# kvas7andy/unreal

Measured on AMD Instinct MI355X. Metric: env-steps/sec (whole node), UNREAL maze 84x84, higher is better.
Workload: dtype f32 (fp16x2-split MFMA operands, fp32 accumulate)

## Files before the change

### include/unreal_hip.h

```cpp
#ifndef UNREAL_HIP_H
#define UNREAL_HIP_H
#include <stdint.h>
#ifdef __cplusplus
extern "C" {
#endif

#define UNREAL_FRAME_BYTES 21168
#define UNREAL_PC_CELLS 400
#define UNREAL_GEMM_RELU 1
#define UNREAL_GEMM_ACCUM 2
#define UNREAL_GEMM_ATOMIC 4
#define UNREAL_GEMM_RELU_MASK 8
#define UNREAL_GEMM_RELU_BITS 16

int unreal_maze_step(int B, int H1, const int* actions, const int* active, int* pos, int* last_action,
                     float* last_reward, int* count, uint8_t* frames, float* r_reward, int* r_action,
                     int* r_terminal, int* r_last_action, float* r_last_reward, float* r_pc,
                     float* out_reward, int* out_terminal, float* episode_reward, float* score_out,
                     int* score_valid, int reset_on_terminal, int track_score, void* stream);
int unreal_maze_rollout_step(int B, int H1, const int* actions, int* pos, int* last_action, float* last_reward, int* count,
                             uint8_t* frames, float* r_reward, int* r_action, int* r_terminal, int* r_last_action,
                             float* r_last_reward, float* r_pc, float* out_reward, int* out_terminal,
                             float* episode_reward, float* score_out, int* score_valid, int* active,
                             int* active_log_t, int* n_steps, int* terminal_end, int* next_idx ,
// ... 162 lines not shown
                       const float* bv, const double* u, float* pi_out, float* v_out, int* action, void* stream);
int unreal_base_loss_grad(int rows, int A, const float* pi, int ld_pi, const float* v, const int* action,
                          const float* adv, const float* R, const int* active, float entropy_beta, float grad_scale,
                          float* dlogits, float* dv, float* losses , void* stream);
int unreal_vr_loss_grad(int rows, const float* v, const float* R, const int* mask, float grad_scale, float* dv,
                        float* loss, void* stream);
int unreal_rp_loss_grad(int rows, const float* logits, const int* cls, float grad_scale, float* prob, float* dlogits,
                        float* loss, void* stream);
int unreal_colsum(int rows, int cols, const float* X, int ld, float* out, void* stream);
int unreal_relu_mask(int rows, int cols, float* d, int ldd, const float* src, int lds, void* stream);

int unreal_pc_deconv_fwd(int N, int A, const float* hp, const float* hp_absmax, const float* Wv, const float* bv,
                         const float* Wa, const float* ba, float* qmax, const int* action, const float* target,
                         const int* mask, float lambda, float grad_scale, float* d_dec, float* ddec_absmax, float* loss,
                         void* stream);
int unreal_pc_deconv_bwd(int N, int A, const float* hp, const float* hp_absmax, const float* d_dec, const float* ddec_absmax,
                         const float* Wv, const float* Wa, float* d_hp, float* dhp_absmax ,
                         float* dWv, float* dbv, float* dWa, float* dba, void* stream);
int unreal_pc_deconv_train(int N, int A, const float* hp, const float* hp_absmax, const float* Wv, const float* bv,
                           const float* Wa, const float* ba, const int* action, const float* target, const int* mask,
                           float lambda, float grad_scale, float* loss, float* d_hp,
                           float* dhp_absmax , float* dWv, float* dbv, float* dWa,
                           float* dba, float* d_dec, void* stream);

int unreal_grad_norm(const float* grad, long n, float* scratch , float* norm_out, void* stream);
int unreal_rmsprop_step(float* var, float* ms, float* mom, const float* grad, long n, float lr, float decay,
                        float momentum, float eps, float clip_norm, const float* norm, void* stream);

int unreal_copy_words(long n, const void* src, void* dst, void* stream);
int unreal_axpy_f32(long n, float alpha, const float* x, float* y, void* stream);
int unreal_last_launch(char* buf, int len, void* stream);

#ifdef __cplusplus
}
#endif
#endif
```

### unreal_amd/csrc/pc.hip

```cpp
#include "common.h"

namespace {

constexpr int HP_LD = 36, HP_ROWS = 84;
constexpr int NPLP = 2;
constexpr int WD_ELEMS = 4 * 4 * 2 * 4 * 16 * 4;
constexpr int HP_V = (C2_POS * 8 + 255) / 256;
constexpr int DD_V = (PC_CELLS * 8 / 4 + 255) / 256;

struct PcFwdArgs {
  int N, A;
  const float* hp;
  const float* hp_absmax;
  const float* Wv; const float* bv; const float* Wa; const float* ba;
  float* qmax;
  const int* action;
  const float* target;
  const int* mask;
  float lambda, grad_scale;
  float* d_dec;
  float* ddec_absmax;
  float* loss;
};

// ... 5 lines not shown
}

__device__ __forceinline__ void hp_load(const float* __restrict__ src, int gtid, f32x4 (&r)[HP_V]) {
  const f32x4* s4 = reinterpret_cast<const f32x4*>(src);
#pragma unroll
  for (int c = 0; c < HP_V; ++c) {
    int id = gtid + 256 * c;
    r[c] = s4[id < C2_POS * 8 ? id : gtid];
  }
}

__device__ __forceinline__ void hp_store(float* hp, int gtid, const f32x4 (&r)[HP_V]) {
#pragma unroll
  for (int c = 0; c < HP_V; ++c) {
    int id = gtid + 256 * c;
    if (id < C2_POS * 8) *reinterpret_cast<f32x4*>(hp + (id >> 3) * HP_LD + (id & 7) * 4) = r[c];
  }
}

typedef _Float16 fh8p __attribute__((ext_vector_type(8)));
typedef _Float16 fh2p __attribute__((ext_vector_type(2)));
typedef float f32x2p __attribute__((ext_vector_type(2)));
typedef unsigned int u32x2p __attribute__((ext_vector_type(2)));

constexpr int HPP_ROW = 80;
constexpr int HPP_PLANE = HP_ROWS * HPP_ROW;
constexpr int WDP_ROW = 80;
constexpr int WDP_PLANE = 4 * 32 * WDP_ROW;

__device__ __forceinline__ void split4p(const f32x4& v, float scale, u32x2p (&pl)[NPLP]) {
  const f32x2p x01 = (f32x2p){v[0], v[1]} * scale, x23 = (f32x2p){v[2], v[3]} * scale;
  const fh2p h01 = __builtin_convertvector(x01, fh2p), h23 = __builtin_convertvector(x23, fh2p);
  const fh2p l01 = __builtin_convertvector(x01 - __builtin_convertvector(h01, f32x2p), fh2p);
  const fh2p l23 = __builtin_convertvector(x23 - __builtin_convertvector(h23, f32x2p), fh2p);
  pl[0] = (u32x2p){__builtin_bit_cast(unsigned int, h01), __builtin_bit_cast(unsigned int, h23)};
  pl[1] = (u32x2p){__builtin_bit_cast(unsigned int, l01), __builtin_bit_cast(unsigned int, l23)};
}

__device__ __forceinline__ void hp_store_planes(unsigned char* hpp, int gtid, const f32x4 (&r)[HP_V], float scale) {
#pragma unroll
  for (int c = 0; c < HP_V; ++c) {
    const int id = gtid + 256 * c;
    if (id < C2_POS * 8) {
      u32x2p pl[NPLP];
      split4p(r[c], scale, pl);
      pl[0][0] = keep_positive_visible(pl[0][0], r[c][0], r[c][1]);
// ... 37 lines not shown
      for (int k = 0; k < 4; ++k) v[k] = deconv_w(Wv, Wa, A, ky, kx, co, 4 * c4 + k);
    }
    u32x2p pl[NPLP];
    split4p(v, S_W, pl);
#pragma unroll
    for (int t = 0; t < NPLP; ++t) *reinterpret_cast<u32x2p*>(wdp + t * WDP_PLANE + (dd * 32 + n) * WDP_ROW + c4 * 8) = pl[t];
  }
}

__device__ __forceinline__ void pc_zero_hp_pad_rows(unsigned char* hpp) {
  for (int e = threadIdx.x; e < NPLP * 3 * HPP_ROW / 4; e += 256) {
    const int t = e / (3 * HPP_ROW / 4), w = e % (3 * HPP_ROW / 4);
    reinterpret_cast<uint32_t*>(hpp + t * HPP_PLANE + C2_POS * HPP_ROW)[w] = 0u;
  }
}

template <int COT> struct FwdLds {
  static constexpr int DS = COT | 1;
  static constexpr int DEC = NPLP * HPP_PLANE, DOUT = DEC + PC_CELLS * DS * 4, W = DOUT + PC_CELLS * COT * 4,
                       BYTES = W + NPLP * WDP_PLANE;
  static constexpr int WGS = 3 * BYTES <= 160 * 1024 ? 3 : 2;
};

template <bool TWO_NT, int DS>
__device__ __forceinline__ void deconv_packed(const unsigned char* hpp, const unsigned char* wdp, float* dec, int mt0, int i,
                                              int q, int CO, const float (&bias)[2], float unscale) {
  constexpr int NTL = TWO_NT ? 2 : 1;
  const int ntiles = (mt0 + 4 < 7) ? 2 : 1;
  f32x4 acc[2][NTL];
  int a[2], b[2];
#pragma unroll
  for (int t = 0; t < 2; ++t) {
#pragma unroll
    for (int nt = 0; nt < NTL; ++nt) acc[t][nt] = (f32x4){0.f, 0.f, 0.f, 0.f};
    const int m = min((mt0 + 4 * t) * 16 + i, 99);
    a[t] = m / 10;
    b[t] = m % 10;
  }
#pragma unroll
  for (int dd = 0; dd < 4; ++dd) {
    const int da = dd >> 1, db = dd & 1;
    fh8p bw[NTL][NPLP];
#pragma unroll
    for (int nt = 0; nt < NTL; ++nt)
#pragma unroll
      for (int pl = 0; pl < NPLP; ++pl)
        bw[nt][pl] = *reinterpret_cast<const fh8p*>(wdp + pl * WDP_PLANE + ((dd * 32 + nt * 16 + i)) * WDP_ROW + 16 * q);
#pragma unroll
    for (int t = 0; t < 2; ++t) {
      if (t < ntiles) {
        const int y = a[t] - da, x = b[t] - db;
        const int row = (y >= 0 && y < 9 && x >= 0 && x < 9) ? y * 9 + x : C2_POS;
        fh8p av[NPLP];
#pragma unroll
        for (int pl = 0; pl < NPLP; ++pl)
          av[pl] = *reinterpret_cast<const fh8p*>(hpp + pl * HPP_PLANE + row * HPP_ROW + 16 * q);
#pragma unroll
        for (int nt = 0; nt < NTL; ++nt) PC_SPLIT_MMA(av, bw[nt], acc[t][nt]);
      }
    }
  }
#pragma unroll
  for (int nt = 0; nt < NTL; ++nt) {
    const int n = nt * 16 + i;
    if (n < 4 * CO) {
      const int par = n / CO, co = n - par * CO;
#pragma unroll
      for (int t = 0; t < 2; ++t)
        if (t < ntiles) {
#pragma unroll
// ... 49 lines not shown
  }
  int prev = -1;
  for (int base = blockIdx.x; base < p.N; base += stride) {
    const int n = base;
    const bool valid = n < p.N;
    const int nn = n + stride;
    const bool has_next = nn < p.N;
    __syncthreads();
    if (prev >= 0 && p.d_dec) {
      f32x4* dst = reinterpret_cast<f32x4*>(p.d_dec + (size_t)prev * PC_CELLS * CO);
      for (int id = gtid; id < PC_CELLS * CO / 4; id += 256) dst[id] = reinterpret_cast<const f32x4*>(dout)[id];
    }
    if (has_next) hp_load(p.hp + (size_t)nn * F2_DIM, gtid, pre);
    float tg[2] = {0.f, 0.f};
    int act = 0;
    bool on = true;
    if (valid && p.d_dec) {
      tg[0] = p.target[(size_t)n * PC_CELLS + gtid];
      tg[1] = p.target[(size_t)n * PC_CELLS + min(gtid + 256, PC_CELLS - 1)];
      act = p.action[n];
      on = p.mask[n] != 0;
    }
    if (valid) {
      if (two_nt) deconv_packed<true, DS>(hpp, wdp, dec, gw, i, q, CO, bias, unscale);
      else deconv_packed<false, DS>(hpp, wdp, dec, gw, i, q, CO, bias, unscale);
    }
    __syncthreads();
    if (valid) {
#pragma unroll
      for (int pi = 0; pi < 2; ++pi) {
        const int pos = gtid + 256 * pi;
        if (pos >= PC_CELLS) break;
        const float* d = dec + pos * DS;
        const float vpre = d[0];
        const float V = fmaxf(vpre, 0.f);
        float adv[8], mean = 0.f;
        for (int k = 0; k < A; ++k) { adv[k] = fmaxf(d[1 + k], 0.f); mean += adv[k]; }
        mean /= (float)A;
        if (p.qmax) {
          float mx = V + adv[0] - mean;
          for (int k = 1; k < A; ++k) mx = fmaxf(mx, V + adv[k] - mean);
          p.qmax[(size_t)n * PC_CELLS + pos] = mx;
        }
        if (p.d_dec) {
          const float qa = V + adv[act] - mean;
          const float diff = tg[pi] - qa;
          const float dq = on ? -p.lambda * diff * p.grad_scale : 0.f;
          if (on) loss_acc += 0.5f * p.lambda * diff * diff;
// ... 67 lines not shown
    const int k = e & 31, ci = (e >> 5) & 31, ky = e >> 10;
    const int kx = k >> 3, co = k & 7;
    float v = 0.f;
    if (co == 0) v = Wv[(ky * 4 + kx) * 32 + ci];
    else if (co <= A) v = Wa[((ky * 4 + kx) * A + (co - 1)) * 32 + ci];
    unsigned short t[NPLP];
    split1p(v, S_W, t);
#pragma unroll
    for (int pl = 0; pl < NPLP; ++pl)
      reinterpret_cast<unsigned short*>(wbp + pl * WBP_PLANE + (ky * 32 + ci) * WDP_ROW)[k] = t[pl];
  }
}

__device__ __forceinline__ void pc_stage_dd(unsigned char* ddp, int gtid, const float (&dd)[2][8], float S_DD, float (&adbk)[8]) {
#pragma unroll
  for (int h = 0; h < 2; ++h) {
    const int pos = gtid + 256 * h;
    if (pos < PC_CELLS) {
      u32x2p lo[NPLP], hi[NPLP];
      split4p((f32x4){dd[h][0], dd[h][1], dd[h][2], dd[h][3]}, S_DD, lo);
      split4p((f32x4){dd[h][4], dd[h][5], dd[h][6], dd[h][7]}, S_DD, hi);
#pragma unroll
      for (int pl = 0; pl < NPLP; ++pl) {
        typedef unsigned int u32x4p __attribute__((ext_vector_type(4)));
        *reinterpret_cast<u32x4p*>(ddp + pl * DDP_PLANE + pos * DDP_ROW) = (u32x4p){lo[pl][0], lo[pl][1], hi[pl][0], hi[pl][1]};
      }
#pragma unroll
      for (int k = 0; k < 8; ++k) adbk[k] += dd[h][k];
    }
  }
}

__device__ __forceinline__ void pc_dgrad_frame(const unsigned char* hpp, const unsigned char* ddp, const unsigned char* wbp,
                                               float* dhs, int gw, int i, int q, float un_dgrad) {
  const int nt = gw & 1;
  f32x4 acc[3];
  int abase[3];
#pragma unroll
  for (int jj = 0; jj < 3; ++jj) {
    acc[jj] = (f32x4){0.f, 0.f, 0.f, 0.f};
    const int pos = min(((gw >> 1) + 2 * jj) * 16 + i, C2_POS - 1);
    abase[jj] = ((2 * (pos / 9)) * 20 + 2 * (pos % 9) + q) * DDP_ROW;
  }
#pragma unroll
  for (int ky = 0; ky < 4; ++ky) {
    fh8p bw[NPLP];
#pragma unroll
    for (int pl = 0; pl < NPLP; ++pl)
      bw[pl] = *reinterpret_cast<const fh8p*>(wbp + pl * WBP_PLANE + (ky * 32 + nt * 16 + i) * WDP_ROW + 16 * q);
#pragma unroll
    for (int jj = 0; jj < 3; ++jj) {
      fh8p av[NPLP];
#pragma unroll
      for (int pl = 0; pl < NPLP; ++pl)
        av[pl] = *reinterpret_cast<const fh8p*>(ddp + pl * DDP_PLANE + abase[jj] + ky * 20 * DDP_ROW);
      PC_SPLIT_MMA(av, bw, acc[jj]);
    }
  }
#pragma unroll
  for (int jj = 0; jj < 3; ++jj)
#pragma unroll
    for (int r = 0; r < 4; ++r) {
      const int pos = ((gw >> 1) + 2 * jj) * 16 + 4 * q + r;
      if (pos < C2_POS) {
        const int ci = nt * 16 + i;
        const unsigned short h0 = reinterpret_cast<const unsigned short*>(hpp + pos * HPP_ROW)[ci];
        dhs[pos * 32 + ci] = (h0 != 0 && !(h0 & 0x8000)) ? acc[jj][r] * un_dgrad : 0.f;
      }
    }
}

__device__ __forceinline__ void pc_wgrad_frame(const unsigned char* hpp, const unsigned char* ddp, int gw, int i, int q,
// ... 111 lines not shown
#pragma unroll
      for (int co = 0; co < 8; ++co) pre_dd[h][co] = (co < CO) ? src[pos * CO + co] : 0.f;
    }
  };

  __syncthreads();
  {
    const int n0 = blockIdx.x;
    if (n0 < p.N) {
      hp_load(p.hp + (size_t)n0 * F2_DIM, gtid, pre_hp);
      hp_store_planes(hpp, gtid, pre_hp, S_HP);
      load_dd(n0);
      pc_stage_dd(ddp, gtid, pre_dd, S_DD, adbk);
    }
  }
  for (int n = blockIdx.x; n < p.N; n += stride) {
    const int nn = n + stride;
    const bool has_next = nn < p.N;
    __syncthreads();
    if (has_next) {
      hp_load(p.hp + (size_t)nn * F2_DIM, gtid, pre_hp);
      load_dd(nn);
    }
    pc_dgrad_frame(hpp, ddp, wbp, dhs, gw, i, q, un_dgrad);
    pc_wgrad_frame(hpp, ddp, gw, i, q, aw);
    __syncthreads();
    dhp_max = pc_drain_dhp(dhs, p.d_hp + (size_t)n * F2_DIM, gtid, dhp_max);
    if (has_next) {
      hp_store_planes(hpp, gtid, pre_hp, S_HP);
      pc_stage_dd(ddp, gtid, pre_dd, S_DD, adbk);
    }
  }
  pc_commit_grads(aw, un_wgrad, adbk, dhp_max, A, p.dWv, p.dWa, p.dbv, p.dba, p.dhp_absmax, s_red, gw, lane, i, q);
}

struct PcTrainArgs {
  int N, A;
  const float* hp; const float* hp_absmax;
  const float* Wv; const float* bv; const float* Wa; const float* ba;
  const int* action; const float* target; const int* mask;
  float lambda, grad_scale;
  float* loss;
  float* d_hp; float* dhp_absmax;
  float* dWv; float* dbv; float* dWa; float* dba;
  float* d_dec;
};

template <int COT> struct TrainLds {
  static constexpr int DS = COT | 1;
  static constexpr int UNI = PC_CELLS * DS * 4 > F2_DIM * 4 ? PC_CELLS * DS * 4 : F2_DIM * 4;
  static constexpr int DDP = NPLP * HPP_PLANE, U = DDP + NPLP * DDP_PLANE, WF = U + UNI, WB = WF + NPLP * WDP_PLANE,
                       RED = WB + NPLP * WBP_PLANE, BYTES = RED + 192;
  static constexpr int WGS = 2 * BYTES <= 160 * 1024 ? 2 : 1;
};

template <int COT>
__global__ __launch_bounds__(256, TrainLds<COT>::WGS) void pc_deconv_train_kernel(PcTrainArgs p) {
  typedef TrainLds<COT> L;
  constexpr int DS = L::DS;
  __shared__ __attribute__((aligned(16))) unsigned char smem[L::BYTES];
  const int gtid = threadIdx.x;
  const int lane = threadIdx.x & 63, gw = gtid >> 6;
  const int i = lane & 15, q = lane >> 4;
  unsigned char* hpp = smem;
  unsigned char* ddp = smem + L::DDP;
  float* uni = reinterpret_cast<float*>(smem + L::U);
  unsigned char* wdp = smem + L::WF;
  unsigned char* wbp = smem + L::WB;
  float* red = reinterpret_cast<float*>(smem + L::RED);
  const int A = p.A, CO = 1 + p.A;

  const float S_W = pow2_scale(pc_weight_max(p.Wv, p.Wa, A, red));
  const float S_HP = pow2_scale(*p.hp_absmax);
  const float un_fwd = pow2_inv(S_HP) * pow2_inv(S_W);
  pc_fwd_weight_planes(p.Wv, p.Wa, A, wdp, S_W);
  pc_bwd_weight_planes(p.Wv, p.Wa, A, wbp, S_W);
  pc_zero_hp_pad_rows(hpp);
  for (int e = gtid; e < NPLP * DDP_PLANE / 4; e += 256) reinterpret_cast<uint32_t*>(ddp)[e] = 0u;
  float bias[2];
#pragma unroll
  for (int nt = 0; nt < 2; ++nt) {
    const int n = nt * 16 + i;
    const int co = n % CO;
    bias[nt] = (n < 4 * CO) ? (co == 0 ? p.bv[0] : p.ba[co - 1]) : 0.f;
  }
  const bool two_nt = 4 * CO > 16;

  f32x4 aw[2][2];
#pragma unroll
  for (int a = 0; a < 2; ++a)
#pragma unroll
    for (int b = 0; b < 2; ++b) aw[a][b] = (f32x4){0.f, 0.f, 0.f, 0.f};
  float adbk[8];
#pragma unroll
  for (int k = 0; k < 8; ++k) adbk[k] = 0.f;
  float dhp_max = 0.f, loss_acc = 0.f;

  const int stride = gridDim.x;
  f32x4 pre[HP_V];
  __syncthreads();
  if (blockIdx.x < p.N) {
    hp_load(p.hp + (size_t)blockIdx.x * F2_DIM, gtid, pre);
    hp_store_planes(hpp, gtid, pre, S_HP);
  }
  for (int n = blockIdx.x; n < p.N; n += stride) {
    const int nn = n + stride;
    const bool has_next = nn < p.N;
    __syncthreads();
    if (has_next) hp_load(p.hp + (size_t)nn * F2_DIM, gtid, pre);
    const float tg[2] = {p.target[(size_t)n * PC_CELLS + gtid], p.target[(size_t)n * PC_CELLS + min(gtid + 256, PC_CELLS - 1)]};
    const int act = p.action[n];
    const bool on = p.mask[n] != 0;
    if (two_nt) deconv_packed<true, DS>(hpp, wdp, uni, gw, i, q, CO, bias, un_fwd);
    else deconv_packed<false, DS>(hpp, wdp, uni, gw, i, q, CO, bias, un_fwd);
    __syncthreads();
    float dd[2][8];
    float fmx = 0.f;
#pragma unroll
    for (int pi = 0; pi < 2; ++pi) {
#pragma unroll
      for (int k = 0; k < 8; ++k) dd[pi][k] = 0.f;
      const int pos = gtid + 256 * pi;
      if (pos < PC_CELLS) {
        const float* d = uni + pos * DS;
        const float vpre = d[0];
        const float V = fmaxf(vpre, 0.f);
        float apre[COT - 1], mean = 0.f, aact = 0.f;
#pragma unroll
        for (int k = 0; k < COT - 1; ++k) {
          apre[k] = k < A ? d[1 + k] : 0.f;
          const float ad = fmaxf(apre[k], 0.f);
          mean += ad;
          aact = (k == act) ? ad : aact;
        }
        mean /= (float)A;
        const float qa = V + aact - mean;
        const float diff = tg[pi] - qa;
        const float dq = on ? -p.lambda * diff * p.grad_scale : 0.f;
        if (on) loss_acc += 0.5f * p.lambda * diff * diff;
        fmx = fmaxf(fmx, fabsf(dq));
        dd[pi][0] = vpre > 0.f ? dq : 0.f;
#pragma unroll
        for (int k = 0; k < COT - 1; ++k)
          dd[pi][1 + k] = (k < A && apre[k] > 0.f) ? dq * (((k == act) ? 1.f : 0.f) - 1.f / (float)A) : 0.f;
        if (p.d_dec) {
          float* o = p.d_dec + ((size_t)n * PC_CELLS + pos) * CO;
#pragma unroll
          for (int k = 0; k < COT; ++k)
            if (k < CO) o[k] = dd[pi][k];
        }
      }
    }
    fmx = wave_max(fmx);
    if (lane == 0) red[40 + gw] = fmx;
    __syncthreads();
    const float S_DD = pow2_scale(fmaxf(fmaxf(red[40], red[41]), fmaxf(red[42], red[43])));
    const float inv_dd = pow2_inv(S_DD);
    pc_stage_dd(ddp, gtid, dd, S_DD, adbk);
    __syncthreads();
    pc_dgrad_frame(hpp, ddp, wbp, uni, gw, i, q, inv_dd * pow2_inv(S_W));
    {
      f32x4 awf[2][2];
#pragma unroll
      for (int a = 0; a < 2; ++a)
#pragma unroll
        for (int b = 0; b < 2; ++b) awf[a][b] = (f32x4){0.f, 0.f, 0.f, 0.f};
      pc_wgrad_frame(hpp, ddp, gw, i, q, awf);
#pragma unroll
      for (int a = 0; a < 2; ++a)
#pragma unroll
        for (int b = 0; b < 2; ++b) aw[a][b] += awf[a][b] * inv_dd;
    }
    __syncthreads();
    dhp_max = pc_drain_dhp(uni, p.d_hp + (size_t)n * F2_DIM, gtid, dhp_max);
    if (has_next) hp_store_planes(hpp, gtid, pre, S_HP);
  }
  __syncthreads();
  loss_acc = wave_sum(loss_acc);
  if (lane == 0) red[44 + gw] = loss_acc;
  pc_commit_grads(aw, pow2_inv(S_HP), adbk, dhp_max, A, p.dWv, p.dWa, p.dbv, p.dba, p.dhp_absmax, red, gw, lane, i, q);
  if (gtid == 0) atomicAdd(p.loss, (((red[44] + red[45]) + red[46]) + red[47]) * p.grad_scale);
}

constexpr int WIDE_CO = UNREAL_MAX_ACTIONS + 1;
constexpr int WIDE_HS_LD = 33;
constexpr int WIDE_HS_BYTES = 82 * WIDE_HS_LD * 4;
constexpr int WIDE_WT_LD = 32 * WIDE_CO;
constexpr int WIDE_WS_BYTES = 16 * WIDE_WT_LD * 4;
constexpr int WIDE_DD_BYTES = PC_CELLS * WIDE_CO * 4;
constexpr int WIDE_WG_ENTRIES = (16 * WIDE_CO + 7) / 8;
constexpr int WIDE_FWD_BYTES = WIDE_HS_BYTES + WIDE_WS_BYTES;
constexpr int WIDE_TRAIN_BYTES = WIDE_FWD_BYTES + WIDE_DD_BYTES;
static_assert(3 * (WIDE_FWD_BYTES + 64) <= 160 * 1024, "three wide forward workgroups must fit one CU's LDS");
static_assert(2 * (WIDE_TRAIN_BYTES + 192) <= 160 * 1024, "two wide training workgroups must fit one CU's LDS");

__device__ __forceinline__ void wide_stage_weights(const float* __restrict__ Wv, const float* __restrict__ Wa, int A,
                                                   float* ws) {
  for (int e = threadIdx.x; e < 16 * 32 * WIDE_CO; e += 256) {
// ... 332 lines not shown
    default: PC_FWD(8); break;
  }
#undef PC_FWD
  return unreal_launch_status();
}

int unreal_pc_deconv_bwd(int N, int A, const float* hp, const float* hp_absmax, const float* d_dec, const float* ddec_absmax,
                         const float* Wv, const float* Wa, float* d_hp, float* dhp_absmax, float* dWv, float* dbv, float* dWa,
                         float* dba, void* stream) {
  if (N <= 0 || A <= 0 || A > UNREAL_MAX_ACTIONS || !hp || !hp_absmax || !d_dec || !ddec_absmax || !Wv || !Wa || !d_hp || !dWv || !dbv ||
      !dWa || !dba)
    return UNREAL_EINVAL;
  if ((((uintptr_t)hp) | ((uintptr_t)d_dec) | ((uintptr_t)d_hp)) & 15) return UNREAL_EINVAL;
  PcBwdArgs p{N, A, hp, hp_absmax, d_dec, ddec_absmax, Wv, Wa, d_hp, dWv, dbv, dWa, dba, dhp_absmax};
  int blocks = min(N, 512);
  if (A > 7) {
    hipLaunchKernelGGL(pc_deconv_bwd_wide_kernel, dim3(blocks), dim3(256), 0, (hipStream_t)stream, p);
    return unreal_launch_status();
  }
  hipLaunchKernelGGL(pc_deconv_bwd_kernel, dim3(blocks), dim3(256), 0, (hipStream_t)stream, p);
  return unreal_launch_status();
}

int unreal_pc_deconv_train(int N, int A, const float* hp, const float* hp_absmax, const float* Wv, const float* bv,
                           const float* Wa, const float* ba, const int* action, const float* target, const int* mask,
                           float lambda, float grad_scale, float* loss, float* d_hp, float* dhp_absmax, float* dWv, float* dbv,
                           float* dWa, float* dba, float* d_dec, void* stream) {
  if (N <= 0 || A <= 0 || A > UNREAL_MAX_ACTIONS || !hp || !hp_absmax || !Wv || !bv || !Wa || !ba || !action || !target ||
      !mask || !loss ||
      !d_hp || !dWv || !dbv || !dWa || !dba)
    return UNREAL_EINVAL;
  if ((((uintptr_t)hp) | ((uintptr_t)d_hp)) & 15) return UNREAL_EINVAL;
  PcTrainArgs p{N, A, hp, hp_absmax, Wv, bv, Wa, ba, action, target, mask, lambda, grad_scale, loss, d_hp, dhp_absmax,
                dWv, dbv, dWa, dba, d_dec};
  hipStream_t st = (hipStream_t)stream;
  if (A > 7) {
    hipLaunchKernelGGL(pc_deconv_train_wide_kernel, dim3(min(N, 256 * 2)), dim3(256), 0, st, p);
    return unreal_launch_status();
  }
#define PC_TRAIN(COT) \
  hipLaunchKernelGGL(pc_deconv_train_kernel<COT>, dim3(min(N, 256 * TrainLds<COT>::WGS)), dim3(256), 0, st, p)
  switch (1 + A) {
    case 4: PC_TRAIN(4); break;
    case 5: PC_TRAIN(5); break;
    case 7: PC_TRAIN(7); break;
    default: PC_TRAIN(8); break;
  }
#undef PC_TRAIN
  return unreal_launch_status();
}

}
```

### unreal_amd/model/model.py

```python
import math
from collections import OrderedDict

import numpy as np
import torch

from .. import ops

ALIGN = 64
XLD = 264


def xcat_ld(action_size, objective_size=0):
    return max(XLD, (256 + action_size + 1 + objective_size + 7) // 8 * 8)


def _small_chunks(n):
    out = []
    while n > 0:
        w = n if n in (1, 3, 4, 5, 6, 7) else (1 if n == 2 else (7 if n >= 10 else n - 3 if n - 3 in (3, 4, 5, 6) else 4))
        out.append(w)
        n -= w
    return out


# ... 195 lines not shown
            K_x = self.K_x
            ss = ops.ShadowSet(self._device, 12)
            S = lambda *a, **k: ss.add(ops.SplitWeights(*a, wmax=ss.slot(), defer=True, **k))
            F = self.F
            sh = dict(fc1_fwd=S(p["W_base_fc1"], F, 256, 256, True),
                      fc1_dgrad=S(p["W_base_fc1"], F, 256, 256, False))
            if self._use_lstm:
                W = p["lstm_kernel"]
                sh.update(lstm_xh_fwd=ss.add(ops.LstmKernelShadow(W, K_x, wmax=ss.slot(), defer=True)),
                          lstm_h_dgrad=S(W, 256, 1024, 1024, False, offset=K_x * 1024),
                          lstm_fc_dgrad=S(W, 256, 1024, 1024, False))
                if self.hoist_lstm_x:
                    sh.update(lstm_x_fwd=S(W, K_x, 1024, 1024, True),
                              lstm_h_fwd=S(W, 256, 1024, 1024, True, offset=K_x * 1024, row_perm=1))
            if self._use_pixel_change:
                sh.update(pc_fc1_fwd=S(p["W_pc_fc1"], 256, 2592, 2592, True),
                          pc_fc1_dgrad=S(p["W_pc_fc1"], 256, 2592, 2592, False))
            self._shadow, self._shadow_set = sh, ss
        self._shadow_set.refresh()
        if self.prepare_encoder and not self.hw:
            p = self.p
            self._enc_prep = ops.encoder_prepare(p["W_base_conv1"], p["b_base_conv1"], p["W_base_conv2"], self.frame_scale,
                                                 self._enc_prep)

    prepare_encoder = True
    _enc_prep = None

    @property
    def enc_prepared(self):
        if not self.prepare_encoder or self.hw:
            return None
        if self._enc_prep is None or self._shadow_stale:
            self.refresh_shadows()
        return self._enc_prep

    @property
    def shadow(self):
        if self._shadow is None:
            self.refresh_shadows()
        return self._shadow

    def _hoist_shadows(self):
        sh = self.shadow
        if "lstm_x_fwd" not in sh:
            ss, W, K_x = self._shadow_set, self.p["lstm_kernel"], self.K_x
            S = lambda *a, **k: ss.add(ops.SplitWeights(*a, wmax=ss.slot(), defer=True, **k))
            sh.update(lstm_x_fwd=S(W, K_x, 1024, 1024, True),
                      lstm_h_fwd=S(W, 256, 1024, 1024, True, offset=K_x * 1024, row_perm=1))
            ss.refresh()
        return sh

    @property
    def ws_kw(self):
        return dict(f2_dim=self.F, c1_dim=self.c1_dim)

    def new_path_ws(self, rows, B, device=None, save_c1=True, lstm=None):
        return PathWS(rows, B, self._device if device is None else device, save_c1=save_c1,
# ... 364 lines not shown
```

### unreal_amd/ops.py

```python
import torch

from ._lib import lib, ptr, stream

FRAME_BYTES = 21168
PC_CELLS = 400
F2_DIM = 2592
C1_DIM = 6400
GEMM_RELU, GEMM_ACCUM, GEMM_ATOMIC, GEMM_RELU_MASK, GEMM_RELU_BITS = 1, 2, 4, 8, 16
RELU_WORDS = 162

FRAME_SHAPE = (84, 84)
FRAME_HW_MIN, FRAME_HW_MAX = 20, 480


def frame_dims(H, W):
    H, W = int(H), int(W)
    if not (FRAME_HW_MIN <= H <= FRAME_HW_MAX and FRAME_HW_MIN <= W <= FRAME_HW_MAX):
        raise ValueError("frame size %dx%d: supported are %d <= H, W <= %d" % (H, W, FRAME_HW_MIN, FRAME_HW_MAX))
    h1, w1 = (H - 8) // 4 + 1, (W - 8) // 4 + 1
    h2, w2 = (h1 - 4) // 2 + 1, (w1 - 4) // 2 + 1
    return h1, w1, h2, w2, 32 * h2 * w2


def frame_stride(H, W):
# ... 765 lines not shown
                  grad_scale=1.0, d_dec=None, loss=None, hp_max=None, ddec_max=None):
    _chk(hp, "f32", N * F2_DIM); _chk(Wv, "f32", 512); _chk(bv, "f32", 1); _chk(Wa, "f32", 512 * A); _chk(ba, "f32", A)
    _chk(qmax, "f32", N * PC_CELLS, optional=True); _chk(action, "i32", N, optional=True)
    _chk(target, "f32", N * PC_CELLS, optional=True); _chk(mask, "i32", N, optional=True)
    _chk(d_dec, "f32", N * PC_CELLS * (1 + A), optional=True); _chk(loss, "f32", 1, optional=True)
    _chk(hp_max, "f32", 1, "hp_max", optional=True); _chk(ddec_max, "f32", 1, "ddec_max", optional=True)
    hp_max = _absmax_of(hp, N, F2_DIM, F2_DIM, hp_max)
    _call("unreal_pc_deconv_fwd", N, A, ptr(hp), ptr(hp_max), ptr(Wv), ptr(bv), ptr(Wa), ptr(ba), ptr(qmax), ptr(action),
          ptr(target), ptr(mask), float(lam), float(grad_scale), ptr(d_dec), ptr(ddec_max), ptr(loss))


def pc_deconv_bwd(N, A, hp, d_dec, Wv, Wa, d_hp, dWv, dbv, dWa, dba, dhp_max=None, hp_max=None, ddec_max=None):
    _chk(hp, "f32", N * F2_DIM); _chk(d_dec, "f32", N * PC_CELLS * (1 + A)); _chk(Wv, "f32", 512)
    _chk(Wa, "f32", 512 * A); _chk(d_hp, "f32", N * F2_DIM); _chk(dWv, "f32", 512); _chk(dbv, "f32", 1)
    _chk(dWa, "f32", 512 * A); _chk(dba, "f32", A)
    _chk(dhp_max, "f32", 1, "dhp_max", optional=True)
    _chk(hp_max, "f32", 1, "hp_max", optional=True); _chk(ddec_max, "f32", 1, "ddec_max", optional=True)
    hp_max = _absmax_of(hp, N, F2_DIM, F2_DIM, hp_max)
    ddec_max = _absmax_of(d_dec, N, PC_CELLS * (1 + A), PC_CELLS * (1 + A), ddec_max)
    _call("unreal_pc_deconv_bwd", N, A, ptr(hp), ptr(hp_max), ptr(d_dec), ptr(ddec_max), ptr(Wv), ptr(Wa), ptr(d_hp),
          ptr(dhp_max), ptr(dWv), ptr(dbv), ptr(dWa), ptr(dba))


def pc_deconv_train(N, A, hp, Wv, bv, Wa, ba, action, target, mask, lam, grad_scale, loss, d_hp, dWv, dbv, dWa, dba,
                    dhp_max=None, hp_max=None, d_dec=None):
    _chk(hp, "f32", N * F2_DIM); _chk(Wv, "f32", 512); _chk(bv, "f32", 1); _chk(Wa, "f32", 512 * A); _chk(ba, "f32", A)
    _chk(action, "i32", N); _chk(target, "f32", N * PC_CELLS); _chk(mask, "i32", N); _chk(loss, "f32", 1)
    _chk(d_hp, "f32", N * F2_DIM); _chk(dWv, "f32", 512); _chk(dbv, "f32", 1); _chk(dWa, "f32", 512 * A); _chk(dba, "f32", A)
    _chk(dhp_max, "f32", 1, "dhp_max", optional=True); _chk(hp_max, "f32", 1, "hp_max", optional=True)
    _chk(d_dec, "f32", N * PC_CELLS * (1 + A), optional=True)
    hp_max = _absmax_of(hp, N, F2_DIM, F2_DIM, hp_max)
    _call("unreal_pc_deconv_train", N, A, ptr(hp), ptr(hp_max), ptr(Wv), ptr(bv), ptr(Wa), ptr(ba), ptr(action), ptr(target),
          ptr(mask), float(lam), float(grad_scale), ptr(loss), ptr(d_hp), ptr(dhp_max), ptr(dWv), ptr(dbv), ptr(dWa), ptr(dba),
          ptr(d_dec))


def axpy(alpha, x, y):
    _chk(x, "f32"); _chk(y, "f32", x.numel())
    _call("unreal_axpy_f32", x.numel(), float(alpha), ptr(x), ptr(y))


def copy_(dst, src):
    if dst.dtype != src.dtype or dst.dtype not in (torch.float32, torch.int32):
        raise ValueError("copy_: %s <- %s" % (dst.dtype, src.dtype))
    if not (dst.is_cuda and src.is_cuda and dst.is_contiguous() and src.is_contiguous()):
        raise ValueError("copy_ needs contiguous device tensors (no CPU fallback)")
    if dst.numel() != src.numel():
        raise ValueError("copy_: %d <- %d elements" % (dst.numel(), src.numel()))
    _call("unreal_copy_words", dst.numel(), ptr(src), ptr(dst))
    return dst


def grad_norm(grad, scratch, norm_out):
    _chk(grad, "f32"); _chk(scratch, "f32", 256); _chk(norm_out, "f32", 1)
    _call("unreal_grad_norm", ptr(grad), grad.numel(), ptr(scratch), ptr(norm_out))


# ... 7 lines not shown
```

### unreal_amd/train/trainer.py

```python
import time

import torch

from .. import ops
from ..environment.environment import Environment
from ..environment.maze_environment import BatchedMazeEnvironment
from ..model.model import UnrealModel, PathWS, GradWS
from .experience import Experience

PERFORMANCE_LOG_INTERVAL = 2000


def log_uniform(lo, hi, rate):
    import math
    return math.exp(math.log(lo) * (1 - rate) + math.log(hi) * rate)


class PhiloxDraws(object):

    def __init__(self, seed, rank=0, batch=None, world_size=1):
        self.seed = int(seed)
        self.counter = 1
        self.batch = None if batch is None else int(batch)
        self.stride = None if batch is None else int(batch) * int(world_size)
# ... 441 lines not shown
        return feat, ld

    def _aux_forward(self):
        B, Ta, net, ws = self.Bg, self.local_t_max, self.local_network, self.aux_ws
        rows = Ta * B
        ops.copy_(ws.frame_idx[:rows], self.seq_idx[:rows])
        if self.use_lstm:
            ws.c0.zero_()
            ws.h0.zero_()
        ops.seq_mask(B, Ta, self.seq_len, self.seq_mask)
        return net.trunk_forward(self.ring, ws, Ta, B, lar_from_ring=True, save_c1=True)

    fuse_pc_deconv = True
    keep_d_dec = False

    def _pc_deconv_loss_backward(self, gws, rows, mask, d_hp, s_hp):
        A, net = self.action_size, self.local_network
        p, g = net.p, net.g
        s_dhp = net.new_slot()
        if self.fuse_pc_deconv:
            ops.pc_deconv_train(rows, A, gws.hp, p["W_pc_deconv_v"], p["b_pc_deconv_v"], p["W_pc_deconv_a"], p["b_pc_deconv_a"],
                                self.seq_act, gws.pc_R, mask, self.pixel_change_lambda, self.grad_scale, self.losses[3:4], d_hp,
                                g["W_pc_deconv_v"], g["b_pc_deconv_v"], g["W_pc_deconv_a"], g["b_pc_deconv_a"], dhp_max=s_dhp,
                                hp_max=s_hp, d_dec=gws.ensure_d_dec(rows, A) if self.keep_d_dec else None)
            return s_dhp
        s_dd = net.new_slot()
        d_dec = gws.ensure_d_dec(rows, A)
        ops.pc_deconv_fwd(rows, A, gws.hp, p["W_pc_deconv_v"], p["b_pc_deconv_v"], p["W_pc_deconv_a"],
                          p["b_pc_deconv_a"], action=self.seq_act, target=gws.pc_R, mask=mask,
                          lam=self.pixel_change_lambda, grad_scale=self.grad_scale, d_dec=d_dec,
                          loss=self.losses[3:4], hp_max=s_hp, ddec_max=s_dd)
        ops.pc_deconv_bwd(rows, A, gws.hp, d_dec, p["W_pc_deconv_v"], p["W_pc_deconv_a"], d_hp,
                          g["W_pc_deconv_v"], g["b_pc_deconv_v"], g["W_pc_deconv_a"], g["b_pc_deconv_a"], dhp_max=s_dhp,
                          hp_max=s_hp, ddec_max=s_dd)
        return s_dhp

    def _train_pc(self):
        B, Ta, A, net = self.Bg, self.local_t_max, self.action_size, self.local_network
        p, g, gws = net.p, net.g, self.gws
        rows = Ta * B
        ws = self.aux_ws
        gws.ensure_pc(rows, A)
        feat, ld = self._sample_sequence()
        s_bhp = net.new_slot()
        net.pc_head_forward(B, feat, ld, self.boot_hp, ws=self.boot_ws, hp_max=s_bhp)
        ops.pc_deconv_fwd(B, A, self.boot_hp, p["W_pc_deconv_v"], p["b_pc_deconv_v"], p["W_pc_deconv_a"],
                          p["b_pc_deconv_a"], qmax=self.boot_qmax, hp_max=s_bhp)
# ... 178 lines not shown
```

Before: 3.712 million.

## Precompute PC deconv weight MFMA fragments once per weight update

Adds a prepare kernel that splits the pixel-change deconv weights into fp16 hi/lo MFMA fragments, computes their scale once when the shadows are refreshed, and passes the result to the fused train kernel. The train kernel copies the forward fragments into a smaller LDS region and reads the backward fragments straight into registers from global memory, so the weight-max reduction and the per-block weight-plane staging are gone. The smaller LDS footprint allows three workgroups per CU instead of two. In exchange it adds an extra kernel launch per weight refresh and more register pressure from holding the backward fragments.

```diff
diff --git a/include/unreal_hip.h b/include/unreal_hip.h
--- a/include/unreal_hip.h
+++ b/include/unreal_hip.h
@@ -208,6 +208,12 @@
                            float lambda, float grad_scale, float* loss, float* d_hp,
                            float* dhp_absmax , float* dWv, float* dbv, float* dWa,
                            float* dba, float* d_dec, void* stream);
+int unreal_pc_deconv_train_prepared(int N, int A, const float* hp, const float* hp_absmax, const float* Wv, const float* bv,
+                                    const float* Wa, const float* ba, const int* action, const float* target, const int* mask,
+                                    float lambda, float grad_scale, float* loss, float* d_hp, float* dhp_absmax, float* dWv,
+                                    float* dbv, float* dWa, float* dba, float* d_dec, const void* prepared, void* stream);
+#define UNREAL_PC_PREPARED_BYTES 32784
+int unreal_pc_prepare(const float* Wv, const float* Wa, int A, void* prepared, long prepared_bytes, void* stream);
 
 int unreal_grad_norm(const float* grad, long n, float* scratch , float* norm_out, void* stream);
 int unreal_rmsprop_step(float* var, float* ms, float* mom, const float* grad, long n, float lr, float decay,
diff --git a/unreal_amd/csrc/pc.hip b/unreal_amd/csrc/pc.hip
--- a/unreal_amd/csrc/pc.hip
+++ b/unreal_amd/csrc/pc.hip
@@ -51,6 +51,7 @@
 typedef _Float16 fh2p __attribute__((ext_vector_type(2)));
 typedef float f32x2p __attribute__((ext_vector_type(2)));
 typedef unsigned int u32x2p __attribute__((ext_vector_type(2)));
+typedef unsigned int u32x4p __attribute__((ext_vector_type(4)));
 
 constexpr int HPP_ROW = 80;
 constexpr int HPP_PLANE = HP_ROWS * HPP_ROW;
@@ -134,8 +135,8 @@
   static constexpr int WGS = 3 * BYTES <= 160 * 1024 ? 3 : 2;
 };
 
-template <bool TWO_NT, int DS>
-__device__ __forceinline__ void deconv_packed(const unsigned char* hpp, const unsigned char* wdp, float* dec, int mt0, int i,
+template <bool TWO_NT, int DS, typename WFrag>
+__device__ __forceinline__ void deconv_packed(const unsigned char* hpp, const WFrag& wfrag, float* dec, int mt0, int i,
                                               int q, int CO, const float (&bias)[2], float unscale) {
   constexpr int NTL = TWO_NT ? 2 : 1;
   const int ntiles = (mt0 + 4 < 7) ? 2 : 1;
@@ -157,7 +158,7 @@
     for (int nt = 0; nt < NTL; ++nt)
 #pragma unroll
       for (int pl = 0; pl < NPLP; ++pl)
-        bw[nt][pl] = *reinterpret_cast<const fh8p*>(wdp + pl * WDP_PLANE + ((dd * 32 + nt * 16 + i)) * WDP_ROW + 16 * q);
+        bw[nt][pl] = wfrag(dd, nt, pl);
 #pragma unroll
     for (int t = 0; t < 2; ++t) {
       if (t < ntiles) {
@@ -253,8 +254,11 @@
       on = p.mask[n] != 0;
     }
     if (valid) {
-      if (two_nt) deconv_packed<true, DS>(hpp, wdp, dec, gw, i, q, CO, bias, unscale);
-      else deconv_packed<false, DS>(hpp, wdp, dec, gw, i, q, CO, bias, unscale);
+      const auto wfrag = [&](int dd, int nt, int pl) {
+        return *reinterpret_cast<const fh8p*>(wdp + pl * WDP_PLANE + (dd * 32 + nt * 16 + i) * WDP_ROW + 16 * q);
+      };
+      if (two_nt) deconv_packed<true, DS>(hpp, wfrag, dec, gw, i, q, CO, bias, unscale);
+      else deconv_packed<false, DS>(hpp, wfrag, dec, gw, i, q, CO, bias, unscale);
     }
     __syncthreads();
     if (valid) {
@@ -368,7 +372,6 @@
       split4p((f32x4){dd[h][4], dd[h][5], dd[h][6], dd[h][7]}, S_DD, hi);
 #pragma unroll
       for (int pl = 0; pl < NPLP; ++pl) {
-        typedef unsigned int u32x4p __attribute__((ext_vector_type(4)));
         *reinterpret_cast<u32x4p*>(ddp + pl * DDP_PLANE + pos * DDP_ROW) = (u32x4p){lo[pl][0], lo[pl][1], hi[pl][0], hi[pl][1]};
       }
 #pragma unroll
@@ -377,7 +380,8 @@
   }
 }
 
-__device__ __forceinline__ void pc_dgrad_frame(const unsigned char* hpp, const unsigned char* ddp, const unsigned char* wbp,
+template <typename WFrag>
+__device__ __forceinline__ void pc_dgrad_frame(const unsigned char* hpp, const unsigned char* ddp, const WFrag& wfrag,
                                                float* dhs, int gw, int i, int q, float un_dgrad) {
   const int nt = gw & 1;
   f32x4 acc[3];
@@ -393,7 +397,7 @@
     fh8p bw[NPLP];
 #pragma unroll
     for (int pl = 0; pl < NPLP; ++pl)
-      bw[pl] = *reinterpret_cast<const fh8p*>(wbp + pl * WBP_PLANE + (ky * 32 + nt * 16 + i) * WDP_ROW + 16 * q);
+      bw[pl] = wfrag(ky, pl);
 #pragma unroll
     for (int jj = 0; jj < 3; ++jj) {
       fh8p av[NPLP];
@@ -551,7 +555,9 @@
       hp_load(p.hp + (size_t)nn * F2_DIM, gtid, pre_hp);
       load_dd(nn);
     }
-    pc_dgrad_frame(hpp, ddp, wbp, dhs, gw, i, q, un_dgrad);
+    pc_dgrad_frame(hpp, ddp, [&](int ky, int pl) {
+      return *reinterpret_cast<const fh8p*>(wbp + pl * WBP_PLANE + (ky * 32 + (gw & 1) * 16 + i) * WDP_ROW + 16 * q);
+    }, dhs, gw, i, q, un_dgrad);
     pc_wgrad_frame(hpp, ddp, gw, i, q, aw);
     __syncthreads();
     dhp_max = pc_drain_dhp(dhs, p.d_hp + (size_t)n * F2_DIM, gtid, dhp_max);
@@ -573,14 +579,69 @@
   float* d_hp; float* dhp_absmax;
   float* dWv; float* dbv; float* dWa; float* dba;
   float* d_dec;
+  const u32x4p* prep;
 };
+
+constexpr int PC_PREP_FWD = 1, PC_PREP_BWD = PC_PREP_FWD + 4 * 2 * NPLP * 64, PC_PREP_VECS = PC_PREP_BWD + 4 * 2 * NPLP * 64;
+constexpr int PC_WF_BYTES = 4 * 2 * NPLP * 64 * 16;
+
+__device__ __forceinline__ void pc_fwd_frag(const float* __restrict__ Wv, const float* __restrict__ Wa, int A, float S_W,
+                                            int dd, int nt, int i, int q, u32x4p (&f)[NPLP]) {
+  const int CO = 1 + A, n = nt * 16 + i;
+  u32x2p pl[2][NPLP];
+#pragma unroll
+  for (int h = 0; h < 2; ++h) {
+    f32x4 v = {0.f, 0.f, 0.f, 0.f};
+    if (n < 4 * CO) {
+      const int par = n / CO, co = n - par * CO;
+      const int ky = (par >> 1) + 2 * (dd >> 1), kx = (par & 1) + 2 * (dd & 1);
+#pragma unroll
+      for (int k = 0; k < 4; ++k) v[k] = deconv_w(Wv, Wa, A, ky, kx, co, 8 * q + 4 * h + k);
+    }
+    split4p(v, S_W, pl[h]);
+  }
+#pragma unroll
+  for (int t = 0; t < NPLP; ++t) f[t] = (u32x4p){pl[0][t][0], pl[0][t][1], pl[1][t][0], pl[1][t][1]};
+}
+
+__device__ __forceinline__ void pc_bwd_frag(const float* __restrict__ Wv, const float* __restrict__ Wa, int A, float S_W,
+                                            int ky, int nt, int i, int q, u32x4p (&f)[NPLP]) {
+  const int ci = nt * 16 + i, kx = q;
+  unsigned short t[8][NPLP];
+#pragma unroll
+  for (int co = 0; co < 8; ++co) {
+    float v = 0.f;
+    if (co == 0) v = Wv[(ky * 4 + kx) * 32 + ci];
+    else if (co <= A) v = Wa[((ky * 4 + kx) * A + (co - 1)) * 32 + ci];
+    split1p(v, S_W, t[co]);
+  }
+#pragma unroll
+  for (int pl = 0; pl < NPLP; ++pl)
+#pragma unroll
+    for (int j = 0; j < 4; ++j) f[pl][j] = (unsigned int)t[2 * j][pl] | ((unsigned int)t[2 * j + 1][pl] << 16);
+}
+
+__global__ __launch_bounds__(256) void pc_prepare_kernel(const float* __restrict__ Wv, const float* __restrict__ Wa, int A,
+                                                         u32x4p* __restrict__ prep) {
+  __shared__ float red;
+  const float S_W = pow2_scale(pc_weight_max(Wv, Wa, A, &red));
+  if (threadIdx.x == 0) prep[0] = (u32x4p){__float_as_uint(S_W), (unsigned int)A, 0u, 0u};
+  for (int e = threadIdx.x; e < 2 * 4 * 2 * 64; e += 256) {
+    const int lane = e & 63, nt = (e >> 6) & 1, step = (e >> 7) & 3, bwd = e >> 9;
+    u32x4p f[NPLP];
+    if (bwd) pc_bwd_frag(Wv, Wa, A, S_W, step, nt, lane & 15, lane >> 4, f);
+    else pc_fwd_frag(Wv, Wa, A, S_W, step, nt, lane & 15, lane >> 4, f);
+#pragma unroll
+    for (int pl = 0; pl < NPLP; ++pl) prep[(bwd ? PC_PREP_BWD : PC_PREP_FWD) + ((step * 2 + nt) * NPLP + pl) * 64 + lane] = f[pl];
+  }
+}
 
 template <int COT> struct TrainLds {
   static constexpr int DS = COT | 1;
   static constexpr int UNI = PC_CELLS * DS * 4 > F2_DIM * 4 ? PC_CELLS * DS * 4 : F2_DIM * 4;
-  static constexpr int DDP = NPLP * HPP_PLANE, U = DDP + NPLP * DDP_PLANE, WF = U + UNI, WB = WF + NPLP * WDP_PLANE,
-                       RED = WB + NPLP * WBP_PLANE, BYTES = RED + 192;
-  static constexpr int WGS = 2 * BYTES <= 160 * 1024 ? 2 : 1;
+  static constexpr int DDP = NPLP * HPP_PLANE, U = DDP + NPLP * DDP_PLANE, WF = U + UNI, RED = WF + PC_WF_BYTES,
+                       BYTES = RED + 192;
+  static constexpr int WGS = 3 * BYTES <= 160 * 1024 ? 3 : 2;
 };
 
 template <int COT>
@@ -594,16 +655,26 @@
   unsigned char* hpp = smem;
   unsigned char* ddp = smem + L::DDP;
   float* uni = reinterpret_cast<float*>(smem + L::U);
-  unsigned char* wdp = smem + L::WF;
-  unsigned char* wbp = smem + L::WB;
+  u32x4p* wf = reinterpret_cast<u32x4p*>(smem + L::WF);
   float* red = reinterpret_cast<float*>(smem + L::RED);
   const int A = p.A, CO = 1 + p.A;
-
-  const float S_W = pow2_scale(pc_weight_max(p.Wv, p.Wa, A, red));
+  const u32x4p* prep = p.prep;
+
+  const float S_W = prep ? __uint_as_float(prep[0][0]) : pow2_scale(pc_weight_max(p.Wv, p.Wa, A, red));
+  for (int e = gtid; e < 4 * 2 * 64; e += 256) {
+    const int nt = (e >> 6) & 1, dd = e >> 7, base = (dd * 2 + nt) * NPLP * 64 + (e & 63);
+    u32x4p f[NPLP];
+    if (prep) {
+#pragma unroll
+      for (int pl = 0; pl < NPLP; ++pl) f[pl] = prep[PC_PREP_FWD + base + pl * 64];
+    } else {
+      pc_fwd_frag(p.Wv, p.Wa, A, S_W, dd, nt, e & 15, (e >> 4) & 3, f);
+    }
+#pragma unroll
+    for (int pl = 0; pl < NPLP; ++pl) wf[base + pl * 64] = f[pl];
+  }
   const float S_HP = pow2_scale(*p.hp_absmax);
   const float un_fwd = pow2_inv(S_HP) * pow2_inv(S_W);
-  pc_fwd_weight_planes(p.Wv, p.Wa, A, wdp, S_W);
-  pc_bwd_weight_planes(p.Wv, p.Wa, A, wbp, S_W);
   pc_zero_hp_pad_rows(hpp);
   for (int e = gtid; e < NPLP * DDP_PLANE / 4; e += 256) reinterpret_cast<uint32_t*>(ddp)[e] = 0u;
   float bias[2];
@@ -635,21 +706,37 @@
   for (int n = blockIdx.x; n < p.N; n += stride) {
     const int nn = n + stride;
     const bool has_next = nn < p.N;
-    __syncthreads();
-    if (has_next) hp_load(p.hp + (size_t)nn * F2_DIM, gtid, pre);
-    const float tg[2] = {p.target[(size_t)n * PC_CELLS + gtid], p.target[(size_t)n * PC_CELLS + min(gtid + 256, PC_CELLS - 1)]};
+    int zero;
+    asm volatile("v_mov_b32 %0, 0" : "=v"(zero));
+    const int ft = gtid + zero, fl = ft & 63, fi = fl & 15, fq = fl >> 4;
+    const auto fwd_frag = [&](int dd, int nt, int pl) {
+      return __builtin_bit_cast(fh8p, wf[((dd * 2 + nt) * NPLP + pl) * 64 + fl]);
+    };
+    __syncthreads();
+    if (has_next) hp_load(p.hp + (size_t)nn * F2_DIM, ft, pre);
+    const float tg[2] = {p.target[(size_t)n * PC_CELLS + ft], p.target[(size_t)n * PC_CELLS + min(ft + 256, PC_CELLS - 1)]};
     const int act = p.action[n];
     const bool on = p.mask[n] != 0;
-    if (two_nt) deconv_packed<true, DS>(hpp, wdp, uni, gw, i, q, CO, bias, un_fwd);
-    else deconv_packed<false, DS>(hpp, wdp, uni, gw, i, q, CO, bias, un_fwd);
-    __syncthreads();
+    if (two_nt) deconv_packed<true, DS>(hpp, fwd_frag, uni, gw, fi, fq, CO, bias, un_fwd);
+    else deconv_packed<false, DS>(hpp, fwd_frag, uni, gw, fi, fq, CO, bias, un_fwd);
+    __syncthreads();
+    u32x4p bwf[4][NPLP];
+#pragma unroll
+    for (int ky = 0; ky < 4; ++ky) {
+      if (prep) {
+#pragma unroll
+        for (int pl = 0; pl < NPLP; ++pl) bwf[ky][pl] = prep[PC_PREP_BWD + ((ky * 2 + (gw & 1)) * NPLP + pl) * 64 + fl];
+      } else {
+        pc_bwd_frag(p.Wv, p.Wa, A, S_W, ky, gw & 1, fi, fq, bwf[ky]);
+      }
+    }
     float dd[2][8];
     float fmx = 0.f;
 #pragma unroll
     for (int pi = 0; pi < 2; ++pi) {
 #pragma unroll
       for (int k = 0; k < 8; ++k) dd[pi][k] = 0.f;
-      const int pos = gtid + 256 * pi;
+      const int pos = ft + 256 * pi;
       if (pos < PC_CELLS) {
         const float* d = uni + pos * DS;
         const float vpre = d[0];
@@ -685,24 +772,25 @@
     __syncthreads();
     const float S_DD = pow2_scale(fmaxf(fmaxf(red[40], red[41]), fmaxf(red[42], red[43])));
     const float inv_dd = pow2_inv(S_DD);
-    pc_stage_dd(ddp, gtid, dd, S_DD, adbk);
-    __syncthreads();
-    pc_dgrad_frame(hpp, ddp, wbp, uni, gw, i, q, inv_dd * pow2_inv(S_W));
+    pc_stage_dd(ddp, ft, dd, S_DD, adbk);
+    __syncthreads();
+    pc_dgrad_frame(hpp, ddp, [&](int ky, int pl) { return __builtin_bit_cast(fh8p, bwf[ky][pl]); }, uni, gw, fi, fq,
+                   inv_dd * pow2_inv(S_W));
     {
       f32x4 awf[2][2];
 #pragma unroll
       for (int a = 0; a < 2; ++a)
 #pragma unroll
         for (int b = 0; b < 2; ++b) awf[a][b] = (f32x4){0.f, 0.f, 0.f, 0.f};
-      pc_wgrad_frame(hpp, ddp, gw, i, q, awf);
+      pc_wgrad_frame(hpp, ddp, gw, fi, fq, awf);
 #pragma unroll
       for (int a = 0; a < 2; ++a)
 #pragma unroll
         for (int b = 0; b < 2; ++b) aw[a][b] += awf[a][b] * inv_dd;
     }
     __syncthreads();
-    dhp_max = pc_drain_dhp(uni, p.d_hp + (size_t)n * F2_DIM, gtid, dhp_max);
-    if (has_next) hp_store_planes(hpp, gtid, pre, S_HP);
+    dhp_max = pc_drain_dhp(uni, p.d_hp + (size_t)n * F2_DIM, ft, dhp_max);
+    if (has_next) hp_store_planes(hpp, ft, pre, S_HP);
   }
   __syncthreads();
   loss_acc = wave_sum(loss_acc);
@@ -1081,17 +1169,17 @@
   return unreal_launch_status();
 }
 
-int unreal_pc_deconv_train(int N, int A, const float* hp, const float* hp_absmax, const float* Wv, const float* bv,
-                           const float* Wa, const float* ba, const int* action, const float* target, const int* mask,
-                           float lambda, float grad_scale, float* loss, float* d_hp, float* dhp_absmax, float* dWv, float* dbv,
-                           float* dWa, float* dba, float* d_dec, void* stream) {
+int unreal_pc_deconv_train_prepared(int N, int A, const float* hp, const float* hp_absmax, const float* Wv, const float* bv,
+                                    const float* Wa, const float* ba, const int* action, const float* target, const int* mask,
+                                    float lambda, float grad_scale, float* loss, float* d_hp, float* dhp_absmax, float* dWv,
+                                    float* dbv, float* dWa, float* dba, float* d_dec, const void* prepared, void* stream) {
   if (N <= 0 || A <= 0 || A > UNREAL_MAX_ACTIONS || !hp || !hp_absmax || !Wv || !bv || !Wa || !ba || !action || !target ||
       !mask || !loss ||
       !d_hp || !dWv || !dbv || !dWa || !dba)
     return UNREAL_EINVAL;
-  if ((((uintptr_t)hp) | ((uintptr_t)d_hp)) & 15) return UNREAL_EINVAL;
+  if ((((uintptr_t)hp) | ((uintptr_t)d_hp) | ((uintptr_t)prepared)) & 15) return UNREAL_EINVAL;
   PcTrainArgs p{N, A, hp, hp_absmax, Wv, bv, Wa, ba, action, target, mask, lambda, grad_scale, loss, d_hp, dhp_absmax,
-                dWv, dbv, dWa, dba, d_dec};
+                dWv, dbv, dWa, dba, d_dec, static_cast<const u32x4p*>(prepared)};
   hipStream_t st = (hipStream_t)stream;
   if (A > 7) {
     hipLaunchKernelGGL(pc_deconv_train_wide_kernel, dim3(min(N, 256 * 2)), dim3(256), 0, st, p);
@@ -1109,4 +1197,19 @@
   return unreal_launch_status();
 }
 
-}
+int unreal_pc_deconv_train(int N, int A, const float* hp, const float* hp_absmax, const float* Wv, const float* bv,
+                           const float* Wa, const float* ba, const int* action, const float* target, const int* mask,
+                           float lambda, float grad_scale, float* loss, float* d_hp, float* dhp_absmax, float* dWv, float* dbv,
+                           float* dWa, float* dba, float* d_dec, void* stream) {
+  return unreal_pc_deconv_train_prepared(N, A, hp, hp_absmax, Wv, bv, Wa, ba, action, target, mask, lambda, grad_scale, loss,
+                                         d_hp, dhp_absmax, dWv, dbv, dWa, dba, d_dec, nullptr, stream);
+}
+
+int unreal_pc_prepare(const float* Wv, const float* Wa, int A, void* prepared, long prepared_bytes, void* stream) {
+  if (!Wv || !Wa || A <= 0 || A > 7 || !prepared || (((uintptr_t)prepared) & 15)) return UNREAL_EINVAL;
+  if (prepared_bytes < (long)PC_PREP_VECS * 16) return UNREAL_EINVAL;
+  hipLaunchKernelGGL(pc_prepare_kernel, dim3(1), dim3(256), 0, (hipStream_t)stream, Wv, Wa, A, static_cast<u32x4p*>(prepared));
+  return unreal_launch_status();
+}
+
+}
diff --git a/unreal_amd/model/model.py b/unreal_amd/model/model.py
--- a/unreal_amd/model/model.py
+++ b/unreal_amd/model/model.py
@@ -241,6 +241,9 @@
             p = self.p
             self._enc_prep = ops.encoder_prepare(p["W_base_conv1"], p["b_base_conv1"], p["W_base_conv2"], self.frame_scale,
                                                  self._enc_prep)
+        if self._use_pixel_change and self._action_size <= 7:
+            p = self.p
+            self._pc_prep = ops.pc_prepare(p["W_pc_deconv_v"], p["W_pc_deconv_a"], self._action_size, self._pc_prep)
 
     prepare_encoder = True
     _enc_prep = None
@@ -252,6 +255,16 @@
         if self._enc_prep is None or self._shadow_stale:
             self.refresh_shadows()
         return self._enc_prep
+
+    _pc_prep = None
+
+    @property
+    def pc_prepared(self):
+        if not self._use_pixel_change or self._action_size > 7:
+            return None
+        if self._pc_prep is None or self._shadow_stale:
+            self.refresh_shadows()
+        return self._pc_prep
 
     @property
     def shadow(self):
diff --git a/unreal_amd/ops.py b/unreal_amd/ops.py
--- a/unreal_amd/ops.py
+++ b/unreal_amd/ops.py
@@ -811,17 +811,30 @@
           ptr(dhp_max), ptr(dWv), ptr(dbv), ptr(dWa), ptr(dba))
 
 
+PC_PREPARED_BYTES = 32784
+
+
+def pc_prepare(Wv, Wa, A, prepared=None):
+    _chk(Wv, "f32", 512); _chk(Wa, "f32", 512 * A)
+    if prepared is None:
+        prepared = torch.empty(PC_PREPARED_BYTES, dtype=torch.uint8, device=Wv.device)
+    _chk(prepared, "u8", PC_PREPARED_BYTES, "prepared")
+    _call("unreal_pc_prepare", ptr(Wv), ptr(Wa), int(A), ptr(prepared), prepared.numel())
+    return prepared
+
+
 def pc_deconv_train(N, A, hp, Wv, bv, Wa, ba, action, target, mask, lam, grad_scale, loss, d_hp, dWv, dbv, dWa, dba,
-                    dhp_max=None, hp_max=None, d_dec=None):
+                    dhp_max=None, hp_max=None, d_dec=None, prepared=None):
     _chk(hp, "f32", N * F2_DIM); _chk(Wv, "f32", 512); _chk(bv, "f32", 1); _chk(Wa, "f32", 512 * A); _chk(ba, "f32", A)
     _chk(action, "i32", N); _chk(target, "f32", N * PC_CELLS); _chk(mask, "i32", N); _chk(loss, "f32", 1)
     _chk(d_hp, "f32", N * F2_DIM); _chk(dWv, "f32", 512); _chk(dbv, "f32", 1); _chk(dWa, "f32", 512 * A); _chk(dba, "f32", A)
     _chk(dhp_max, "f32", 1, "dhp_max", optional=True); _chk(hp_max, "f32", 1, "hp_max", optional=True)
     _chk(d_dec, "f32", N * PC_CELLS * (1 + A), optional=True)
+    _chk(prepared, "u8", PC_PREPARED_BYTES, "prepared", optional=True)
     hp_max = _absmax_of(hp, N, F2_DIM, F2_DIM, hp_max)
-    _call("unreal_pc_deconv_train", N, A, ptr(hp), ptr(hp_max), ptr(Wv), ptr(bv), ptr(Wa), ptr(ba), ptr(action), ptr(target),
-          ptr(mask), float(lam), float(grad_scale), ptr(loss), ptr(d_hp), ptr(dhp_max), ptr(dWv), ptr(dbv), ptr(dWa), ptr(dba),
-          ptr(d_dec))
+    _call("unreal_pc_deconv_train_prepared", N, A, ptr(hp), ptr(hp_max), ptr(Wv), ptr(bv), ptr(Wa), ptr(ba), ptr(action),
+          ptr(target), ptr(mask), float(lam), float(grad_scale), ptr(loss), ptr(d_hp), ptr(dhp_max), ptr(dWv), ptr(dbv),
+          ptr(dWa), ptr(dba), ptr(d_dec), ptr(prepared))
 
 
 def axpy(alpha, x, y):
diff --git a/unreal_amd/train/trainer.py b/unreal_amd/train/trainer.py
--- a/unreal_amd/train/trainer.py
+++ b/unreal_amd/train/trainer.py
@@ -487,7 +487,8 @@
             ops.pc_deconv_train(rows, A, gws.hp, p["W_pc_deconv_v"], p["b_pc_deconv_v"], p["W_pc_deconv_a"], p["b_pc_deconv_a"],
                                 self.seq_act, gws.pc_R, mask, self.pixel_change_lambda, self.grad_scale, self.losses[3:4], d_hp,
                                 g["W_pc_deconv_v"], g["b_pc_deconv_v"], g["W_pc_deconv_a"], g["b_pc_deconv_a"], dhp_max=s_dhp,
-                                hp_max=s_hp, d_dec=gws.ensure_d_dec(rows, A) if self.keep_d_dec else None)
+                                hp_max=s_hp, d_dec=gws.ensure_d_dec(rows, A) if self.keep_d_dec else None,
+                                prepared=net.pc_prepared)
             return s_dhp
         s_dd = net.new_slot()
         d_dec = gws.ensure_d_dec(rows, A)
```

After: 3.733 million (median of 6 runs). About the same (+0.6%).
